# SkyTNT/midi-model

Hardware: AMD Instinct MI355X
Metric: MIDI events/sec, training step (fwd+bwd+clip+AdamW), tv2o-medium, seq=2048 (higher is better)
Workload: dtype bf16; 1 GPU; tv2o-medium bf16 training step, per-GPU batch 16 x 2048 events x 8 tokens (BASELINE.json configs[1]); random-init weights, synthetic events; global_batch=16, seq_len=2048, parallelism=dp1, accumulate_grad_batches=1, optimizer=AdamW bf16-true + global-norm clip 1.0

## Files before the change

### midi-model_amd/csrc/api.cpp

```cpp
#include <stdarg.h>
#include <stdio.h>

#include "../../include/midihip.h"

static thread_local char g_err[512] = "";

void mh_set_error(const char* fmt, ...) {
  va_list ap;
  va_start(ap, fmt);
  vsnprintf(g_err, sizeof(g_err), fmt, ap);
  va_end(ap);
}

#include <stdlib.h>
#include <string.h>
static int env_int(const char* name, int dflt) {
  const char* v = getenv(name);
  return (v && *v) ? atoi(v) : dflt;
}
thread_local int g_mh_gemm_variant = env_int("MH_GEMM", 1);
thread_local int g_mh_gemm_ablate = 0;
thread_local int g_mh_gemm_k64 = env_int("MH_GEMM_K64", 1);
thread_local int g_mh_gemm_lean_epi = env_int("MH_GEMM_LEAN_EPI", 1);
extern thread_local int g_skinny_mb, g_skinny_nbt;
extern thread_local int g_tokattn_bwd_batched;
extern thread_local int g_attn_v3, g_attn_v3_wps, g_attn_passes;

extern "C" int mh_set_option(const char* name, int value) {
  if (strcmp(name, "gemm") == 0) {
    g_mh_gemm_variant = value;
    return 0;
  }
  if (strcmp(name, "gemm_ablate") == 0) {
    g_mh_gemm_ablate = value;
    return 0;
  }
  if (strcmp(name, "gemm_k64") == 0) {
    g_mh_gemm_k64 = value;
    return 0;
  }
  if (strcmp(name, "gemm_lean_epi") == 0) {
    g_mh_gemm_lean_epi = value;
    return 0;
  }
  if (strcmp(name, "tokattn_bwd_batched") == 0) {
    g_tokattn_bwd_batched = value;
    return 0;
  }
  if (strcmp(name, "skinny_mb") == 0) {
    g_skinny_mb = value;
    return 0;
  }
  if (strcmp(name, "attn_v3") == 0) {
    g_attn_v3 = value;
    return 0;
  }
  if (strcmp(name, "attn_passes") == 0) {
    g_attn_passes = value;
    return 0;
  }
  if (strcmp(name, "attn_v3_wps") == 0) {
    g_attn_v3_wps = value;
    return 0;
  }
  if (strcmp(name, "skinny_nbt") == 0) {
    g_skinny_nbt = value;
    return 0;
  }
  mh_set_error("unknown option %s", name);
  return MH_ERR_ARG;
}
extern "C" int mh_get_option(const char* name) {
  if (strcmp(name, "gemm") == 0) return g_mh_gemm_variant;
  if (strcmp(name, "skinny_mb") == 0) return g_skinny_mb;
  if (strcmp(name, "attn_v3") == 0) return g_attn_v3;
  if (strcmp(name, "attn_v3_wps") == 0) return g_attn_v3_wps;
  if (strcmp(name, "attn_passes") == 0) return g_attn_passes;
  if (strcmp(name, "skinny_nbt") == 0) return g_skinny_nbt;
  if (strcmp(name, "gemm_k64") == 0) return g_mh_gemm_k64;
  if (strcmp(name, "gemm_ablate") == 0) return g_mh_gemm_ablate;
  if (strcmp(name, "gemm_lean_epi") == 0) return g_mh_gemm_lean_epi;
  if (strcmp(name, "tokattn_bwd_batched") == 0) return g_tokattn_bwd_batched;
  return -1;
}

extern "C" const char* mh_last_error(void) { return g_err; }
extern "C" int mh_version(void) { return 1; }
extern "C" int mh_ab_builds(void) {
#ifdef MH_AB_BUILDS
  return 1;
#else
  return 0;
#endif
}
```

### midi-model_amd/csrc/gemm_pp256.hip

```cpp
#include <limits.h>

#include <type_traits>

#include "common.h"

namespace {

__device__ __attribute__((aligned(16))) char g_zero16[16];

constexpr int QBM = 256, QBN = 256, QBK = 32;
constexpr int OP_BYTES = 256 * 64;
constexpr int STAGE_BYTES = 2 * OP_BYTES;
constexpr int NSTAGE = 4;
constexpr int LDS_BYTES = NSTAGE * STAGE_BYTES;
constexpr int NWAVE = 8;
constexpr int NI = 2;

typedef __attribute__((ext_vector_type(4))) short s16x4_t;

__device__ inline int tswz(int krow) { return (krow & 3) | ((krow >> 1) & 4); }
__device__ inline int xswz(int row) { return (0x1230 >> (((row >> 2) & 3) * 4)) & 3; }

struct StageCtx {
  const bf16* p[NI];
// ... 50 lines not shown
__device__ inline __amdgpu_buffer_rsrc_t tile_rsrc(const void* base, int64_t bytes) {
  const unsigned n = bytes <= 0 ? 0u : (bytes > 0xfffffff0ll ? 0xfffffff0u : (unsigned)bytes);
  const uint64_t b = (uint64_t)(uintptr_t)base;
  const uint64_t bu = (uint64_t)(unsigned)__builtin_amdgcn_readfirstlane((int)(unsigned)b) |
                      ((uint64_t)(unsigned)__builtin_amdgcn_readfirstlane((int)(unsigned)(b >> 32)) << 32);
  return __builtin_amdgcn_make_buffer_rsrc(reinterpret_cast<void*>((uintptr_t)bu), 0, (unsigned)__builtin_amdgcn_readfirstlane((int)n), 0x00020000);
}
template <int AUX>
__device__ inline void tile_store_(const u32x4& v, __amdgpu_buffer_rsrc_t r, unsigned voff) {
  __builtin_amdgcn_raw_buffer_store_b128(v, r, voff, 0, AUX);
}
#define tile_store(v, r, voff, aux) tile_store_<aux>(v, r, voff)
__device__ inline u32x4 as_u32x4(const bf16x8& v) {
  union {
    bf16x8 b;
    u32x4 u;
  } x;
  x.b = v;
  return x.u;
}
__device__ inline bf16x8 as_bf16x8(const u32x4& v) {
  union {
    bf16x8 b;
    u32x4 u;
  } x;
  x.u = v;
  return x.b;
}

constexpr int P8_REGION = 128 * 128;
constexpr int P8_BUF = 4 * P8_REGION;
constexpr int P8_DBG_BYTES = 8 * 2048;

template <int EPI, int ABL, bool TB>
__device__ __forceinline__ void p8_main_loop(char* smem, const bf16* __restrict__ A, int64_t lda, const bf16* __restrict__ B,
                                             int64_t ldb, int64_t M, int64_t N, int64_t m0, int64_t n0, int64_t kbeg, int64_t kend,
                                             int wave, int lane, const void* __restrict__ zero16, f32x4 (&acc)[4][8]) {
  constexpr bool TL = (ABL & 128) != 0;
  constexpr int LA = 7;
  const int grp = wave >> 2, wn = wave & 3;
  const int fi = lane & 15, fg = lane >> 4;
  const int nt = (kend > kbeg) ? (int)((kend - kbeg + 63) / 64) : 0;
  const int nreg = 4 * nt;

  int tl_n = 0;
  auto stamp = [&]() {
    if constexpr (TL) {
      const uint64_t c = __builtin_readcyclecounter();
      if (lane == 0 && tl_n < 252) *reinterpret_cast<uint64_t*>(smem + 2 * P8_BUF + wave * 2048 + tl_n * 8) = c;
      ++tl_n;
    }
  };
  auto mark = [&](int slot) {
    if constexpr (TL) {
      const uint64_t c = __builtin_readcyclecounter();
      if (lane == 0) *reinterpret_cast<uint64_t*>(smem + 2 * P8_BUF + wave * 2048 + slot * 8) = c;
    }
  };
  mark(252);

  const bf16* pa[2];
  const bf16* pb[2];
  int kla[2][2], klb[2][2];
  const int64_t hoff_a = 64 * lda, hoff_b = TB ? 32 * ldb : (EPI == 2) ? (N / 2) * ldb : 32 * ldb;
#pragma unroll
  for (int it = 0; it < 2; ++it) {
    const int lr = (wave * 2 + it) * 8 + (lane >> 3);
    const int ch = (lane & 7) ^ ((lr >> 1) & 7);
    const int64_t ra = m0 + (lr >> 6) * 128 + (lr & 63);
    pa[it] = A + (ra < M ? ra : 0) * lda + ch * 8;
    kla[0][it] = (ra < M) ? (int)kend - ch * 8 : INT_MIN;
    kla[1][it] = (ra + 64 < M) ? (int)kend - ch * 8 : INT_MIN;
    if constexpr (TB) {
      const int krow = (wave + NWAVE * it) * 2 + (lane >> 5), pc = lane & 31;
      const int lg = (pc >> 1) ^ tswz(krow);
      const int64_t r = n0 + lg * 16 + (pc & 1) * 8;
      pb[it] = B + (int64_t)krow * ldb + (r < N ? r : 0);
      klb[0][it] = (r < N) ? (int)kend - krow : INT_MIN;
      klb[1][it] = (r < N) ? (int)kend - krow - 32 : INT_MIN;
    } else {
      constexpr bool PERM = (EPI == 2 || EPI == 3);
      const int lrp = PERM ? ((lr & ~31) | (((lr & 15) >> 2) << 3) | (((lr >> 4) & 1) << 2) | (lr & 3)) : lr;
      const int64_t rb = (EPI == 2) ? n0 + lrp : n0 + (lrp >> 5) * 64 + (lrp & 31);
      const int64_t rb1 = (EPI == 2) ? rb + N / 2 : rb + 32;
      pb[it] = B + (rb < N ? rb : 0) * ldb + ch * 8;
      klb[0][it] = (rb < N) ? (int)kend - ch * 8 : INT_MIN;
      klb[1][it] = (rb1 < N) ? (int)kend - ch * 8 : INT_MIN;
    }
  }
  auto issue = [&](int s) {
    const int t = s >> 2, r = s & 3;
    const bool isb = (r == 1 || r == 2);
    const int h = (r >= 2) ? 1 : 0;
    const int slot = isb ? 2 + h : h;
    const int k0 = (int)kbeg + t * 64;
#pragma unroll
    for (int it = 0; it < 2; ++it) {
      const int piece = (TB && isb) ? wave + NWAVE * it : wave * 2 + it;
      char* dst = smem + (t & 1) * P8_BUF + slot * P8_REGION + piece * 1024;
      const bf16* p = isb ? pb[it] + (h ? hoff_b : 0) : pa[it] + (h ? hoff_a : 0);
      const int kl = isb ? klb[h][it] : kla[h][it];
      const void* src = (k0 < kl) ? (const void*)((TB && isb) ? p + (int64_t)k0 * ldb : p + k0) : zero16;
      glds16(src, dst);
    }
  };

  const int sw = (fi >> 1) & 7;
  const int la0 = (grp * 64 + fi) * 128 + ((fg ^ sw) << 4);
  const int lb0 = 2 * P8_REGION + (wn * 32 + fi) * 128 + ((fg ^ sw) << 4);
  bf16x8 fx[4][2], fw[2][2][2];
  auto read_a = [&](const char* buf, int mh) {
    if ((ABL & 2) && buf != smem) return;
#pragma unroll
    for (int m4 = 0; m4 < 4; ++m4)
#pragma unroll
      for (int kb = 0; kb < 2; ++kb)
        fx[m4][kb] = *reinterpret_cast<const bf16x8*>(buf + mh * P8_REGION + m4 * 2048 + (la0 ^ (kb << 6)));
  };
  auto read_b = [&](const char* buf, int nh) {
    if ((ABL & 2) && buf != smem) return;
#pragma unroll
    for (int n2 = 0; n2 < 2; ++n2)
#pragma unroll
      for (int kb = 0; kb < 2; ++kb) {
        if constexpr (TB) fw[nh][n2][kb] = frag<true>(buf + (2 + kb) * P8_REGION, wn * 64 + nh * 32 + n2 * 16, fi, fg);
        else fw[nh][n2][kb] = *reinterpret_cast<const bf16x8*>(buf + nh * P8_REGION + n2 * 2048 + (lb0 ^ (kb << 6)));
      }
  };
  auto mfma_q = [&](int mh, int nh) {
#pragma unroll
    for (int kb = 0; kb < 2; ++kb)
#pragma unroll
      for (int n2 = 0; n2 < 2; ++n2)
#pragma unroll
        for (int m4 = 0; m4 < 4; ++m4)
          if (!(ABL & 4))
            acc[nh * 2 + n2][mh * 4 + m4] =
                __builtin_amdgcn_mfma_f32_16x16x32_bf16(fw[nh][n2][kb], fx[m4][kb], acc[nh * 2 + n2][mh * 4 + m4], 0, 0, 0);
  };
  auto bar = [&]() {
    __builtin_amdgcn_sched_barrier(0);
    __builtin_amdgcn_s_barrier();
    __builtin_amdgcn_sched_barrier(0);
  };
  auto wait_lds = [&]() {
    asm volatile("s_waitcnt lgkmcnt(0)" ::: "memory");
    __builtin_amdgcn_sched_barrier(0);
  };
  auto wait_out = [&](int out) {
    if (out >= 4) asm volatile("s_waitcnt vmcnt(8)" ::: "memory");
    else if (out == 3) asm volatile("s_waitcnt vmcnt(6)" ::: "memory");
    else if (out == 2) asm volatile("s_waitcnt vmcnt(4)" ::: "memory");
    else if (out == 1) asm volatile("s_waitcnt vmcnt(2)" ::: "memory");
    else asm volatile("s_waitcnt vmcnt(0)" ::: "memory");
  };
  auto need = [&](int q) { return (q >> 1) * 4 + ((q & 1) ? 4 : 3); };
  auto issued_after = [&](int q) {
    const int n = (q >> 1) * 4 + ((q & 1) ? 11 : 8);
    return n < nreg ? n : nreg;
  };
  auto issue_phase = [&](int q, auto steady) {
    constexpr bool ST = decltype(steady)::value;
    if (!(ABL & 1)) {
      const int t4 = (q >> 1) * 4;
      if ((q & 1) == 0) {
        if (ST || t4 + 7 < nreg) issue(t4 + 7);
      } else {
#pragma unroll
        for (int j = 8; j < 11; ++j)
          if (ST || t4 + j < nreg) issue(t4 + j);
      }
    }
    stamp();
  };
  auto read_phase = [&](int t, int p) {
    const char* buf = smem + (t & 1) * P8_BUF;
    if (p == 0) {
      read_b(buf, 0);
      read_b(buf, 1);
      read_a(buf, 0);
    } else {
      read_a(buf, 1);
    }
    stamp();
  };
  auto load_slot = [&](int t, int p, auto steady) {
    read_phase(t, p);
    issue_phase(2 * t + p, steady);
    wait_lds();
    stamp();
  };
  auto mfma_phase = [&](int p) {
    mfma_q(p, 0);
    mfma_q(p, 1);
    stamp();
  };
  auto wait_next = [&](int q, auto steady) {
    if constexpr (decltype(steady)::value) asm volatile("s_waitcnt vmcnt(8)" ::: "memory");
    else if (q + 1 < 2 * nt) wait_out(issued_after(q) - need(q + 1));
    stamp();
  };
  auto tile_g0 = [&](int t, auto steady) {
#pragma unroll
    for (int p = 0; p < 2; ++p) {
      stamp();
      load_slot(t, p, steady);
      bar();
      stamp();
      mfma_phase(p);
      wait_next(2 * t + p, steady);
      bar();
    }
  };
  auto tile_g1 = [&](int t, auto steady) {
#pragma unroll
    for (int p = 0; p < 2; ++p) {
      stamp();
      if (2 * t + p > 0) mfma_phase(p ^ 1);
      else stamp();
      bar();
      stamp();
      load_slot(t, p, steady);
      wait_next(2 * t + p, steady);
      bar();
    }
  };

#pragma unroll
  for (int s = 0; s < LA; ++s)
    if (s < nreg) issue(s);
  if (nt > 0) wait_out((nreg < LA ? nreg : LA) - need(0));
  bar();
  mark(253);
  const int nsteady = nt > 2 ? nt - 2 : 0;
  if (grp == 0) {
    for (int t = 0; t < nsteady; ++t) tile_g0(t, std::true_type{});
    for (int t = nsteady; t < nt; ++t) tile_g0(t, std::false_type{});
  } else {
    for (int t = 0; t < nsteady; ++t) tile_g1(t, std::true_type{});
    for (int t = nsteady; t < nt; ++t) tile_g1(t, std::false_type{});
    if (nt > 0) mfma_phase(1);
  }
  mark(254);
  if constexpr (TL) {
    asm volatile("s_waitcnt lgkmcnt(0)" ::: "memory");
  }
}

constexpr int GRP_MAX = 8;
struct GrpProblem {
  const bf16* A;
  const bf16* B;
  bf16* C;
  const bf16* R;
  const bf16* wnorm;
  const bf16* W;
  float* colpart;
  int64_t lda, ldb, ldc, ldr, ldw, M, N;
  float alpha, beta;
  int tile0, tiles_n;
};
struct GrpTable {
  GrpProblem p[GRP_MAX];
  int n, nitems;
};
__host__ __device__ inline int xcd_item_of(int lin, int nitems) {
  const int q = nitems >> 3, r8 = nitems & 7, xcd = lin & 7;
  return (xcd < r8 ? xcd * (q + 1) : r8 * (q + 1) + (xcd - r8) * q) + (lin >> 3);
}
__host__ __device__ inline int grp_item_of(const GrpTable& t, int lin, int& tm, int& tn) {
  const int item = xcd_item_of(lin, t.nitems);
  int pi = 0;
#pragma unroll
  for (int j = 1; j < GRP_MAX; ++j)
    if (j < t.n && item >= t.p[j].tile0) pi = j;
  const int tiles_n = t.p[pi].tiles_n;
  const int tiles_m = (int)((t.p[pi].M + QBM - 1) / QBM);
  gemm_tile_of(item - t.p[pi].tile0, tiles_m, tiles_n, 4, tm, tn);
  return pi;
}
template <bool GRP>
struct GrpArg {
  typedef int type;
};
template <>
struct GrpArg<true> {
  typedef GrpTable type;
};

template <bool TA, bool TB, int ABL, int EPI, int ML, int NRM, bool GRP = false>
__global__ __launch_bounds__(512, 2) void gemm_pp256_kernel(const bf16* __restrict__ A, int64_t lda,
                                                            const bf16* __restrict__ B, int64_t ldb, bf16* C, int64_t ldc,
                                                            const bf16* R, int64_t ldr, int64_t M, int64_t N, int64_t K,
                                                            float alpha, float beta, int tiles_n, int nwg,
                                                            int64_t k_per_split, float* __restrict__ ws,
                                                            const void* __restrict__ zero16, float* aux, int lean_epi,
                                                            const typename GrpArg<GRP>::type gtab) {
  static_assert(NRM == 0 || (ML == 1 && ABL == 0 && !TA && (!TB || (EPI == 1 && NRM == 2))), "the norm forms ride on the K-step-64 loops only");
  static_assert(NRM != 1 || EPI == 0, "sum-of-squares partials come out of the plain epilogue");
  static_assert(!GRP || (TA && TB && ABL == 0 && EPI == 0 && ML == 0 && NRM == 0), "the grouped launch is the weight-gradient form");
  extern __shared__ __attribute__((aligned(16))) char smem[];
  const int tid = threadIdx.x, lane = tid & 63;
  const int wave = __builtin_amdgcn_readfirstlane(tid >> 6);
  const int grp = wave >> 2;
  const int wn = wave & 3;

  int zslice = 0, tm, tn;
  const bf16 *wnorm = nullptr, *Wf = nullptr;
  float* colpart = nullptr;
  int64_t ldw = 0;
  if constexpr (GRP) {
    const GrpProblem& P = gtab.p[grp_item_of(gtab, (int)blockIdx.x, tm, tn)];
    A = P.A, lda = P.lda, B = P.B, ldb = P.ldb, C = P.C, ldc = P.ldc, R = P.R, ldr = P.ldr, M = P.M, N = P.N;
    alpha = P.alpha, beta = P.beta;
    wnorm = P.wnorm, Wf = P.W, ldw = P.ldw, colpart = P.colpart;
  } else {
    const int nitems = nwg * (int)gridDim.z;
    const int lin = blockIdx.x + nwg * (int)blockIdx.z;
    const int item = xcd_item_of(lin, nitems);
    zslice = item / nwg;
    gemm_tile_of(item - zslice * nwg, nwg / tiles_n, tiles_n, 4, tm, tn);
  }
// ... 80 lines not shown
    else asm volatile("s_waitcnt vmcnt(0)" ::: "memory");
  };
  auto load_segment = [&](int t) {
    load_frags(t);
    if (t + 3 < nt && !(ABL & 1)) {
#pragma unroll
      for (int j = 0; j < 4; ++j) issue_one(t + 3, j);
    }
    asm volatile("s_waitcnt lgkmcnt(0)" ::: "memory");
    __builtin_amdgcn_sched_barrier(0);
  };
  constexpr bool MIDBAR = ((ABL & 64) != 0) == (TA || TB);
  if (grp == 0) {
    for (int t = 0; t < nt; ++t) {
      wait_step(t);
      bar();
      load_segment(t);
      if (MIDBAR) bar();
      mfma_all(t);
    }
    bar();
  } else {
    for (int t = 0; t < nt; ++t) {
      wait_step(t);
      bar();
      if (t > 0) mfma_all(t - 1);
      if (MIDBAR) bar();
      load_segment(t);
    }
    bar();
    if (nt > 0) mfma_all(nt - 1);
  }
  }

  float rs[8];
  if constexpr (NRM == 2) {
    const float* rl = reinterpret_cast<const float*>(smem + LDS_BYTES);
#pragma unroll
    for (int fm = 0; fm < 8; ++fm) rs[fm] = rl[grp * 128 + fm * 16 + fi];
  }
  const bool partial = (gridDim.z > 1);
  float* wsz = partial ? ws + (int64_t)zslice * M * N : nullptr;
  if constexpr ((ABL & 32) != 0) {
    if (acc[0][0][0] != 1.2345e38f) return;
  }
  if constexpr (EPI == 1) {
    if (lean_epi && m0 + QBM <= M && n0 + QBN <= N && ldc < (1 << 22) && ldr < (1 << 22)) {
      char* wreg = smem + wave * 16384;
      const int lrow = lane >> 3, c = lane & 7;
      const __amdgpu_buffer_rsrc_t rg = tile_rsrc(R + m0 * ldr + n0 + wn * 64, (255 * ldr + N + 64) * 2);
      const __amdgpu_buffer_rsrc_t rc = tile_rsrc(C + m0 * ldc + n0 + wn * 64, (255 * ldc + N + 64) * 2);
      const unsigned vo_r = (unsigned)(((grp * 128 + lrow) * (int)ldr + c * 8) * 2), so_r = (unsigned)ldr * 16u;
      const unsigned vo_c = (unsigned)(((grp * 128 + lrow) * (int)ldc + c * 8) * 2), so_c = (unsigned)ldc * 16u;
      const unsigned up_off = (unsigned)N * 2u;
      bf16x8 gq[2][8], uq[2][8];
      auto request = [&](int half, int i0) {
#pragma unroll
        for (int i = i0; i < i0 + 4; ++i) {
          gq[half][i] = as_bf16x8(__builtin_amdgcn_raw_buffer_load_b128(rg, vo_r, (unsigned)(half * 8 + i) * so_r, 0));
          uq[half][i] = as_bf16x8(__builtin_amdgcn_raw_buffer_load_b128(rg, vo_r, (unsigned)(half * 8 + i) * so_r + up_off, 0));
        }
      };
      request(0, 0);
      request(0, 4);
#pragma unroll
      for (int half = 0; half < 2; ++half) {
#pragma unroll
        for (int fmh = 0; fmh < 4; ++fmh)
#pragma unroll
          for (int fn = 0; fn < 4; ++fn) {
// ... 572 lines not shown
      if (partial) {
        float* dst = wsz + m * N + n;
        if (vec_ok && n + 3 < N) {
          *reinterpret_cast<f32x4*>(dst) = v;
        } else {
          for (int e = 0; e < 4 && n + e < N; ++e) dst[e] = v[e];
        }
        continue;
      }
      if (vec_ok && n + 3 < N) {
        if (R != nullptr && beta != 0.f) {
          bf16x4 rv = *reinterpret_cast<const bf16x4*>(R + m * ldr + n);
#pragma unroll
          for (int e = 0; e < 4; ++e) v[e] = alpha * v[e] + beta * (float)rv[e];
        } else {
#pragma unroll
          for (int e = 0; e < 4; ++e) v[e] = alpha * v[e];
        }
        bf16x4 o;
#pragma unroll
        for (int e = 0; e < 4; ++e) o[e] = (bf16)v[e];
        *reinterpret_cast<bf16x4*>(C + m * ldc + n) = o;
      } else {
        for (int e = 0; e < 4 && n + e < N; ++e) {
          float x = alpha * v[e];
          if (R != nullptr && beta != 0.f) x += beta * (float)R[m * ldr + n + e];
          C[m * ldc + n + e] = (bf16)x;
        }
      }
    }
  }
}

}
extern thread_local int g_mh_gemm_lean_epi;
namespace {
template <auto KERNEL>
int launch_prepare(int LDSB, void** zero16_out) {
  constexpr int MAX_DEV = 64;
  static void* zero16_of[MAX_DEV] = {};
  static bool attr_set_of[MAX_DEV] = {};
  int dev = 0;
  if (hipGetDevice(&dev) != hipSuccess || dev < 0 || dev >= MAX_DEV) {
    mh_set_error("gemm_pp256: no current device (or ordinal %d beyond %d)", dev, MAX_DEV - 1);
    return MH_ERR_LAUNCH;
  }
  void* zero16 = __atomic_load_n(&zero16_of[dev], __ATOMIC_ACQUIRE);
  if (zero16 == nullptr) {
    if (hipGetSymbolAddress(&zero16, HIP_SYMBOL(g_zero16)) != hipSuccess) {
      mh_set_error("gemm_pp256: hipGetSymbolAddress(g_zero16) failed");
      return MH_ERR_LAUNCH;
    }
    __atomic_store_n(&zero16_of[dev], zero16, __ATOMIC_RELEASE);
  }
  if (!__atomic_load_n(&attr_set_of[dev], __ATOMIC_ACQUIRE)) {
    hipError_t e = hipFuncSetAttribute(reinterpret_cast<const void*>(KERNEL), hipFuncAttributeMaxDynamicSharedMemorySize, LDSB);
    if (e != hipSuccess) {
      mh_set_error("gemm_pp256: cannot raise dynamic LDS to %d bytes: %s", LDSB, hipGetErrorString(e));
      return MH_ERR_LAUNCH;
    }
    __atomic_store_n(&attr_set_of[dev], true, __ATOMIC_RELEASE);
  }
  *zero16_out = zero16;
  return MH_OK;
}

template <bool TA, bool TB, int ABL, int EPI = 0, int ML = 0, int NRM = 0>
int launch_one(const void* A, int64_t lda, const void* B, int64_t ldb, void* C, int64_t ldc, const void* R, int64_t ldr,
               int64_t M, int64_t N, int64_t K, float alpha, float beta, int splitk, void* workspace, hipStream_t st,
               float* aux = nullptr) {
  constexpr int LDSB = LDS_BYTES + ((ABL & 128) ? P8_DBG_BYTES : 0) + (NRM == 2 ? 1024 : 0);
  void* zero16 = nullptr;
  if (int rc = launch_prepare<&gemm_pp256_kernel<TA, TB, ABL, EPI, ML, NRM>>(LDSB, &zero16)) return rc;
  const int64_t tiles_m = (M + QBM - 1) / QBM, tiles_n = (EPI == 2) ? N / 256 : (N + QBN - 1) / QBN;
  const int nwg = (int)(tiles_m * tiles_n);
  constexpr int KSTEP = (ML == 1) ? 64 : QBK;
  const int64_t kps = ((K + splitk - 1) / splitk + KSTEP - 1) / KSTEP * KSTEP;
  dim3 grid(nwg, 1, splitk);
  gemm_pp256_kernel<TA, TB, ABL, EPI, ML, NRM><<<grid, 512, LDSB, st>>>((const bf16*)A, lda, (const bf16*)B, ldb, (bf16*)C, ldc,
                                                          (const bf16*)R, ldr, M, N, K, alpha, beta, (int)tiles_n, nwg, kps,
                                                          (float*)workspace, zero16, aux, g_mh_gemm_lean_epi, 0);
  MH_LAUNCH_CHECK();
  return MH_OK;
}

void grp_table_of(const mh_wgrad_problem* p, int n, GrpTable& t) {
  t.n = n;
  int tile0 = 0;
  for (int j = 0; j < GRP_MAX; ++j) {
    GrpProblem& g = t.p[j];
    if (j >= n) {
      g = GrpProblem{};
      g.tile0 = INT_MAX;
      continue;
    }
    g.A = (const bf16*)p[j].dz, g.lda = p[j].lddz, g.B = (const bf16*)p[j].x, g.ldb = p[j].ldx;
    g.C = (bf16*)p[j].dw, g.ldc = p[j].lddw, g.R = (const bf16*)p[j].R, g.ldr = p[j].ldr;
    g.wnorm = (const bf16*)p[j].wnorm, g.W = (const bf16*)p[j].W, g.ldw = p[j].ldw, g.colpart = p[j].colpart;
    g.M = p[j].N, g.N = p[j].K_out, g.alpha = p[j].alpha, g.beta = p[j].beta;
    g.tile0 = tile0;
    g.tiles_n = (int)((g.N + QBN - 1) / QBN);
    tile0 += (int)((g.M + QBM - 1) / QBM) * g.tiles_n;
  }
  t.nitems = tile0;
}
// ... 156 lines not shown
```

Before: 366,800 events/s.

## Add persistent 256x256 GEMM kernel that prefetches the next tile during epilogue

Adds a persistent variant of the pp256 GEMM that launches one workgroup per CU and loops over tiles. While a tile's epilogue runs through a small per-wave LDS staging region, the global-to-LDS loads for the next tile are already issued, and the vmcnt waits are adjusted to count the epilogue stores still in flight. The aim is to hide the epilogue and per-tile launch/prologue latency behind the next tile's loads. It is enabled by default for selected EPI/TB/K classes, with an environment switch to turn it off. The cost is extra LDS use, more complicated waitcnt accounting, and possible load imbalance when the tile count is not a multiple of the CU count.

```diff
diff --git a/midi-model_amd/csrc/api.cpp b/midi-model_amd/csrc/api.cpp
--- a/midi-model_amd/csrc/api.cpp
+++ b/midi-model_amd/csrc/api.cpp
@@ -22,6 +22,8 @@
 thread_local int g_mh_gemm_ablate = 0;
 thread_local int g_mh_gemm_k64 = env_int("MH_GEMM_K64", 1);
 thread_local int g_mh_gemm_lean_epi = env_int("MH_GEMM_LEAN_EPI", 1);
+thread_local int g_mh_gemm_persist = env_int("MH_GEMM_PERSIST", 1);
+thread_local int g_mh_gemm_persist_wgs = env_int("MH_GEMM_PERSIST_WGS", 0);
 extern thread_local int g_skinny_mb, g_skinny_nbt;
 extern thread_local int g_tokattn_bwd_batched;
 extern thread_local int g_attn_v3, g_attn_v3_wps, g_attn_passes;
@@ -41,6 +43,14 @@
   }
   if (strcmp(name, "gemm_lean_epi") == 0) {
     g_mh_gemm_lean_epi = value;
+    return 0;
+  }
+  if (strcmp(name, "gemm_persist") == 0) {
+    g_mh_gemm_persist = value;
+    return 0;
+  }
+  if (strcmp(name, "gemm_persist_wgs") == 0) {
+    g_mh_gemm_persist_wgs = value;
     return 0;
   }
   if (strcmp(name, "tokattn_bwd_batched") == 0) {
@@ -80,6 +90,8 @@
   if (strcmp(name, "gemm_k64") == 0) return g_mh_gemm_k64;
   if (strcmp(name, "gemm_ablate") == 0) return g_mh_gemm_ablate;
   if (strcmp(name, "gemm_lean_epi") == 0) return g_mh_gemm_lean_epi;
+  if (strcmp(name, "gemm_persist") == 0) return g_mh_gemm_persist;
+  if (strcmp(name, "gemm_persist_wgs") == 0) return g_mh_gemm_persist_wgs;
   if (strcmp(name, "tokattn_bwd_batched") == 0) return g_tokattn_bwd_batched;
   return -1;
 }
diff --git a/midi-model_amd/csrc/gemm_pp256.hip b/midi-model_amd/csrc/gemm_pp256.hip
--- a/midi-model_amd/csrc/gemm_pp256.hip
+++ b/midi-model_amd/csrc/gemm_pp256.hip
@@ -106,68 +106,55 @@
 constexpr int P8_BUF = 4 * P8_REGION;
 constexpr int P8_DBG_BYTES = 8 * 2048;
 
-template <int EPI, int ABL, bool TB>
-__device__ __forceinline__ void p8_main_loop(char* smem, const bf16* __restrict__ A, int64_t lda, const bf16* __restrict__ B,
-                                             int64_t ldb, int64_t M, int64_t N, int64_t m0, int64_t n0, int64_t kbeg, int64_t kend,
-                                             int wave, int lane, const void* __restrict__ zero16, f32x4 (&acc)[4][8]) {
-  constexpr bool TL = (ABL & 128) != 0;
-  constexpr int LA = 7;
-  const int grp = wave >> 2, wn = wave & 3;
-  const int fi = lane & 15, fg = lane >> 4;
-  const int nt = (kend > kbeg) ? (int)((kend - kbeg + 63) / 64) : 0;
-  const int nreg = 4 * nt;
-
-  int tl_n = 0;
-  auto stamp = [&]() {
-    if constexpr (TL) {
-      const uint64_t c = __builtin_readcyclecounter();
-      if (lane == 0 && tl_n < 252) *reinterpret_cast<uint64_t*>(smem + 2 * P8_BUF + wave * 2048 + tl_n * 8) = c;
-      ++tl_n;
-    }
-  };
-  auto mark = [&](int slot) {
-    if constexpr (TL) {
-      const uint64_t c = __builtin_readcyclecounter();
-      if (lane == 0) *reinterpret_cast<uint64_t*>(smem + 2 * P8_BUF + wave * 2048 + slot * 8) = c;
-    }
-  };
-  mark(252);
-
+constexpr int P8_LA = 7;
+
+template <int EPI, bool TB>
+struct P8Feed {
+  char* smem;
+  const void* zero16;
   const bf16* pa[2];
   const bf16* pb[2];
   int kla[2][2], klb[2][2];
-  const int64_t hoff_a = 64 * lda, hoff_b = TB ? 32 * ldb : (EPI == 2) ? (N / 2) * ldb : 32 * ldb;
-#pragma unroll
-  for (int it = 0; it < 2; ++it) {
-    const int lr = (wave * 2 + it) * 8 + (lane >> 3);
-    const int ch = (lane & 7) ^ ((lr >> 1) & 7);
-    const int64_t ra = m0 + (lr >> 6) * 128 + (lr & 63);
-    pa[it] = A + (ra < M ? ra : 0) * lda + ch * 8;
-    kla[0][it] = (ra < M) ? (int)kend - ch * 8 : INT_MIN;
-    kla[1][it] = (ra + 64 < M) ? (int)kend - ch * 8 : INT_MIN;
-    if constexpr (TB) {
-      const int krow = (wave + NWAVE * it) * 2 + (lane >> 5), pc = lane & 31;
-      const int lg = (pc >> 1) ^ tswz(krow);
-      const int64_t r = n0 + lg * 16 + (pc & 1) * 8;
-      pb[it] = B + (int64_t)krow * ldb + (r < N ? r : 0);
-      klb[0][it] = (r < N) ? (int)kend - krow : INT_MIN;
-      klb[1][it] = (r < N) ? (int)kend - krow - 32 : INT_MIN;
-    } else {
-      constexpr bool PERM = (EPI == 2 || EPI == 3);
-      const int lrp = PERM ? ((lr & ~31) | (((lr & 15) >> 2) << 3) | (((lr >> 4) & 1) << 2) | (lr & 3)) : lr;
-      const int64_t rb = (EPI == 2) ? n0 + lrp : n0 + (lrp >> 5) * 64 + (lrp & 31);
-      const int64_t rb1 = (EPI == 2) ? rb + N / 2 : rb + 32;
-      pb[it] = B + (rb < N ? rb : 0) * ldb + ch * 8;
-      klb[0][it] = (rb < N) ? (int)kend - ch * 8 : INT_MIN;
-      klb[1][it] = (rb1 < N) ? (int)kend - ch * 8 : INT_MIN;
-    }
-  }
-  auto issue = [&](int s) {
+  int64_t hoff_a, hoff_b, ldb;
+  int kbeg, wave;
+
+  __device__ __forceinline__ void init(char* smem_, const bf16* __restrict__ A, int64_t lda, const bf16* __restrict__ B, int64_t ldb_,
+                                       int64_t M, int64_t N, int64_t m0, int64_t n0, int64_t kbeg_, int64_t kend, int wave_, int lane,
+                                       const void* __restrict__ zero16_) {
+    smem = smem_, zero16 = zero16_, ldb = ldb_, kbeg = (int)kbeg_, wave = wave_;
+    hoff_a = 64 * lda, hoff_b = TB ? 32 * ldb : (EPI == 2) ? (N / 2) * ldb : 32 * ldb;
+#pragma unroll
+    for (int it = 0; it < 2; ++it) {
+      const int lr = (wave * 2 + it) * 8 + (lane >> 3);
+      const int ch = (lane & 7) ^ ((lr >> 1) & 7);
+      const int64_t ra = m0 + (lr >> 6) * 128 + (lr & 63);
+      pa[it] = A + (ra < M ? ra : 0) * lda + ch * 8;
+      kla[0][it] = (ra < M) ? (int)kend - ch * 8 : INT_MIN;
+      kla[1][it] = (ra + 64 < M) ? (int)kend - ch * 8 : INT_MIN;
+      if constexpr (TB) {
+        const int krow = (wave + NWAVE * it) * 2 + (lane >> 5), pc = lane & 31;
+        const int lg = (pc >> 1) ^ tswz(krow);
+        const int64_t r = n0 + lg * 16 + (pc & 1) * 8;
+        pb[it] = B + (int64_t)krow * ldb + (r < N ? r : 0);
+        klb[0][it] = (r < N) ? (int)kend - krow : INT_MIN;
+        klb[1][it] = (r < N) ? (int)kend - krow - 32 : INT_MIN;
+      } else {
+        constexpr bool PERM = (EPI == 2 || EPI == 3);
+        const int lrp = PERM ? ((lr & ~31) | (((lr & 15) >> 2) << 3) | (((lr >> 4) & 1) << 2) | (lr & 3)) : lr;
+        const int64_t rb = (EPI == 2) ? n0 + lrp : n0 + (lrp >> 5) * 64 + (lrp & 31);
+        const int64_t rb1 = (EPI == 2) ? rb + N / 2 : rb + 32;
+        pb[it] = B + (rb < N ? rb : 0) * ldb + ch * 8;
+        klb[0][it] = (rb < N) ? (int)kend - ch * 8 : INT_MIN;
+        klb[1][it] = (rb1 < N) ? (int)kend - ch * 8 : INT_MIN;
+      }
+    }
+  }
+  __device__ __forceinline__ void issue(int s) const {
     const int t = s >> 2, r = s & 3;
     const bool isb = (r == 1 || r == 2);
     const int h = (r >= 2) ? 1 : 0;
     const int slot = isb ? 2 + h : h;
-    const int k0 = (int)kbeg + t * 64;
+    const int k0 = kbeg + t * 64;
 #pragma unroll
     for (int it = 0; it < 2; ++it) {
       const int piece = (TB && isb) ? wave + NWAVE * it : wave * 2 + it;
@@ -177,7 +164,53 @@
       const void* src = (k0 < kl) ? (const void*)((TB && isb) ? p + (int64_t)k0 * ldb : p + k0) : zero16;
       glds16(src, dst);
     }
-  };
+  }
+};
+
+template <int EPI, bool TB>
+__device__ __forceinline__ void p8_prefetch(char* smem, const bf16* __restrict__ A, int64_t lda, const bf16* __restrict__ B, int64_t ldb,
+                                            int64_t M, int64_t N, int64_t m0, int64_t n0, int64_t K, int wave, int lane,
+                                            const void* __restrict__ zero16) {
+  P8Feed<EPI, TB> feed;
+  feed.init(smem, A, lda, B, ldb, M, N, m0, n0, 0, K, wave, lane, zero16);
+  const int nreg = 4 * (int)((K + 63) / 64);
+#pragma unroll
+  for (int s = 0; s < P8_LA; ++s)
+    if (s < nreg) feed.issue(s);
+}
+
+template <int EPI, int ABL, bool TB, int EV = -1>
+__device__ __forceinline__ void p8_main_loop(char* smem, const bf16* __restrict__ A, int64_t lda, const bf16* __restrict__ B,
+                                             int64_t ldb, int64_t M, int64_t N, int64_t m0, int64_t n0, int64_t kbeg, int64_t kend,
+                                             int wave, int lane, const void* __restrict__ zero16, f32x4 (&acc)[4][8],
+                                             bool behind = false) {
+  constexpr bool TL = (ABL & 128) != 0;
+  constexpr int LA = P8_LA;
+  static_assert(EV < 0 || (ABL == 0 && 8 + EV < 64), "vmcnt is a 6-bit count");
+  const int grp = wave >> 2, wn = wave & 3;
+  const int fi = lane & 15, fg = lane >> 4;
+  const int nt = (kend > kbeg) ? (int)((kend - kbeg + 63) / 64) : 0;
+  const int nreg = 4 * nt;
+
+  int tl_n = 0;
+  auto stamp = [&]() {
+    if constexpr (TL) {
+      const uint64_t c = __builtin_readcyclecounter();
+      if (lane == 0 && tl_n < 252) *reinterpret_cast<uint64_t*>(smem + 2 * P8_BUF + wave * 2048 + tl_n * 8) = c;
+      ++tl_n;
+    }
+  };
+  auto mark = [&](int slot) {
+    if constexpr (TL) {
+      const uint64_t c = __builtin_readcyclecounter();
+      if (lane == 0) *reinterpret_cast<uint64_t*>(smem + 2 * P8_BUF + wave * 2048 + slot * 8) = c;
+    }
+  };
+  mark(252);
+
+  P8Feed<EPI, TB> feed;
+  feed.init(smem, A, lda, B, ldb, M, N, m0, n0, kbeg, kend, wave, lane, zero16);
+  auto issue = [&](int s) { feed.issue(s); };
 
   const int sw = (fi >> 1) & 7;
   const int la0 = (grp * 64 + fi) * 128 + ((fg ^ sw) << 4);
@@ -221,7 +254,17 @@
     asm volatile("s_waitcnt lgkmcnt(0)" ::: "memory");
     __builtin_amdgcn_sched_barrier(0);
   };
-  auto wait_out = [&](int out) {
+  auto wait_out = [&](int out, bool extra = false) {
+    if constexpr (EV > 0) {
+      if (extra) {
+        if (out >= 4) asm volatile("s_waitcnt vmcnt(%0)" ::"n"(8 + EV) : "memory");
+        else if (out == 3) asm volatile("s_waitcnt vmcnt(%0)" ::"n"(6 + EV) : "memory");
+        else if (out == 2) asm volatile("s_waitcnt vmcnt(%0)" ::"n"(4 + EV) : "memory");
+        else if (out == 1) asm volatile("s_waitcnt vmcnt(%0)" ::"n"(2 + EV) : "memory");
+        else asm volatile("s_waitcnt vmcnt(%0)" ::"n"(EV) : "memory");
+        return;
+      }
+    }
     if (out >= 4) asm volatile("s_waitcnt vmcnt(8)" ::: "memory");
     else if (out == 3) asm volatile("s_waitcnt vmcnt(6)" ::: "memory");
     else if (out == 2) asm volatile("s_waitcnt vmcnt(4)" ::: "memory");
@@ -270,8 +313,9 @@
     stamp();
   };
   auto wait_next = [&](int q, auto steady) {
-    if constexpr (decltype(steady)::value) asm volatile("s_waitcnt vmcnt(8)" ::: "memory");
-    else if (q + 1 < 2 * nt) wait_out(issued_after(q) - need(q + 1));
+    const bool extra = EV > 0 && behind && q < 2;
+    if constexpr (decltype(steady)::value) wait_out(4, extra);
+    else if (q + 1 < 2 * nt) wait_out(issued_after(q) - need(q + 1), extra);
     stamp();
   };
   auto tile_g0 = [&](int t, auto steady) {
@@ -300,10 +344,12 @@
     }
   };
 
-#pragma unroll
-  for (int s = 0; s < LA; ++s)
-    if (s < nreg) issue(s);
-  if (nt > 0) wait_out((nreg < LA ? nreg : LA) - need(0));
+  if constexpr (EV < 0) {
+#pragma unroll
+    for (int s = 0; s < LA; ++s)
+      if (s < nreg) issue(s);
+  }
+  if (nt > 0) wait_out((nreg < LA ? nreg : LA) - need(0), EV > 0 && behind);
   bar();
   mark(253);
   const int nsteady = nt > 2 ? nt - 2 : 0;
@@ -362,6 +408,12 @@
   typedef GrpTable type;
 };
 
+template <int EPI, int ABL, int ML, int NRM, bool GRP>
+__device__ __forceinline__ void pp256_epilogue(char* smem, const float* rl, f32x4 (&acc)[4][8], bf16* C, int64_t ldc, const bf16* R,
+                                               int64_t ldr, int64_t M, int64_t N, float alpha, float beta, int64_t m0, int64_t n0, int tm,
+                                               int zslice, float* __restrict__ ws, float* aux, int lean_epi, int wave, int lane,
+                                               const bf16* wnorm, const bf16* Wf, int64_t ldw, float* colpart);
+
 template <bool TA, bool TB, int ABL, int EPI, int ML, int NRM, bool GRP = false>
 __global__ __launch_bounds__(512, 2) void gemm_pp256_kernel(const bf16* __restrict__ A, int64_t lda,
                                                             const bf16* __restrict__ B, int64_t ldb, bf16* C, int64_t ldc,
@@ -508,10 +560,19 @@
     if (nt > 0) mfma_all(nt - 1);
   }
   }
-
+  pp256_epilogue<EPI, ABL, ML, NRM, GRP>(smem, reinterpret_cast<const float*>(smem + LDS_BYTES), acc, C, ldc, R, ldr, M, N, alpha, beta, m0, n0,
+                                         tm, zslice, ws, aux, lean_epi, wave, lane, wnorm, Wf, ldw, colpart);
+}
+
+template <int EPI, int ABL, int ML, int NRM, bool GRP>
+__device__ __forceinline__ void pp256_epilogue(char* smem, const float* rl, f32x4 (&acc)[4][8], bf16* C, int64_t ldc, const bf16* R,
+                                               int64_t ldr, int64_t M, int64_t N, float alpha, float beta, int64_t m0, int64_t n0, int tm,
+                                               int zslice, float* __restrict__ ws, float* aux, int lean_epi, int wave, int lane,
+                                               const bf16* wnorm, const bf16* Wf, int64_t ldw, float* colpart) {
+  const int grp = wave >> 2, wn = wave & 3;
+  const int fi = lane & 15, fg = lane >> 4;
   float rs[8];
   if constexpr (NRM == 2) {
-    const float* rl = reinterpret_cast<const float*>(smem + LDS_BYTES);
 #pragma unroll
     for (int fm = 0; fm < 8; ++fm) rs[fm] = rl[grp * 128 + fm * 16 + fi];
   }
@@ -1150,8 +1211,333 @@
   }
 }
 
+constexpr int P8_TURN_LO = P8_BUF + P8_REGION;
+constexpr int P8_TURN_HI = LDS_BYTES;
+constexpr int P8_RSTD = LDS_BYTES + P8_REGION;
+constexpr int P8_PERSIST_LDS = P8_RSTD + 2048;
+template <int EPI, int NRM>
+constexpr int p8_epi_stores() {
+  return EPI == 1 ? 32 : EPI == 2 ? 24 : (EPI == 0 && NRM == 1) ? 32 : 16;
+}
+
+template <int EPI, int NRM>
+__device__ __forceinline__ void p8_epilogue_turn4k(char* wreg, const float* rl, f32x4 (&acc)[4][8], bf16* C, int64_t ldc, const bf16* R,
+                                                   int64_t ldr, int64_t M, int64_t N, float alpha, float beta, int64_t m0, int64_t n0,
+                                                   float* aux, int wave, int lane) {
+  const int grp = wave >> 2, wn = wave & 3;
+  const int fi = lane & 15, fg = lane >> 4;
+  float rs[8];
+  if constexpr (NRM == 2) {
+#pragma unroll
+    for (int fm = 0; fm < 8; ++fm) rs[fm] = rl[grp * 128 + fm * 16 + fi];
+  }
+  auto put_f32 = [&](int fm) {
+#pragma unroll
+    for (int fn = 0; fn < 4; ++fn) {
+      const int ch = fn * 4 + fg;
+      f32x4 t4 = acc[fn][fm];
+      if constexpr (NRM == 2) t4 *= rs[fm];
+      *reinterpret_cast<f32x4*>(wreg + fi * 256 + ((ch ^ fi) << 4)) = t4;
+    }
+  };
+  if constexpr (EPI == 1) {
+    const int lrow = lane >> 3, c = lane & 7;
+    const __amdgpu_buffer_rsrc_t rg = tile_rsrc(R + m0 * ldr + n0 + wn * 64, (255 * ldr + N + 64) * 2);
+    const __amdgpu_buffer_rsrc_t rc = tile_rsrc(C + m0 * ldc + n0 + wn * 64, (255 * ldc + N + 64) * 2);
+    const unsigned vo_r = (unsigned)(((grp * 128 + lrow) * (int)ldr + c * 8) * 2), so_r = (unsigned)ldr * 16u;
+    const unsigned vo_c = (unsigned)(((grp * 128 + lrow) * (int)ldc + c * 8) * 2), so_c = (unsigned)ldc * 16u;
+    const unsigned up_off = (unsigned)N * 2u;
+    bf16x8 gq[16], uq[16];
+    auto request = [&](int i0) {
+#pragma unroll
+      for (int i = i0; i < i0 + 4; ++i) {
+        gq[i] = as_bf16x8(__builtin_amdgcn_raw_buffer_load_b128(rg, vo_r, (unsigned)i * so_r, 0));
+        uq[i] = as_bf16x8(__builtin_amdgcn_raw_buffer_load_b128(rg, vo_r, (unsigned)i * so_r + up_off, 0));
+      }
+    };
+    request(0);
+    request(4);
+#pragma unroll
+    for (int fm = 0; fm < 8; ++fm) {
+      put_f32(fm);
+#pragma unroll
+      for (int i2 = 0; i2 < 2; ++i2) {
+        const int i = fm * 2 + i2, row = i2 * 8 + lrow;
+        if (i == 2) request(8);
+        if (i == 6) request(12);
+        const f32x4 lo = *reinterpret_cast<const f32x4*>(wreg + row * 256 + (((2 * c) ^ row) << 4));
+        const f32x4 hi = *reinterpret_cast<const f32x4*>(wreg + row * 256 + (((2 * c + 1) ^ row) << 4));
+        const float v[8] = {lo[0], lo[1], lo[2], lo[3], hi[0], hi[1], hi[2], hi[3]};
+        float dv[8], g[8], u[8], dg[8], du[8];
+        expand8_bf16(cvt8_bf16(v), dv);
+        expand8_bf16(gq[i], g);
+        expand8_bf16(uq[i], u);
+        mh_dswiglu8(dv, g, u, dg, du);
+        const unsigned so = (unsigned)i * so_c;
+        tile_store(as_u32x4(cvt8_bf16(dg)), rc, vo_c + so, 2 );
+        tile_store(as_u32x4(cvt8_bf16(du)), rc, vo_c + so + up_off, 2);
+      }
+    }
+  } else if constexpr (EPI == 2) {
+    const int64_t I = N >> 1, colw = n0 + wn * 32;
+    bf16* act = const_cast<bf16*>(R);
+    const __amdgpu_buffer_rsrc_t ra = tile_rsrc(act + m0 * ldr + colw, (255 * ldr + 32) * 2);
+    const __amdgpu_buffer_rsrc_t rc = tile_rsrc(C + m0 * ldc + colw, (255 * ldc + I + 32) * 2);
+    const int r4 = lane >> 2, c4 = lane & 3;
+    const unsigned vo_a = (unsigned)(((grp * 128 + r4) * (int)ldr + c4 * 8) * 2), so_a = (unsigned)ldr * 32u;
+    const unsigned vo_c = (unsigned)(((grp * 128 + r4) * (int)ldc + c4 * 8) * 2), so_c = (unsigned)ldc * 32u;
+#pragma unroll
+    for (int fm = 0; fm < 8; ++fm) {
+      float gf[8], uf[8];
+#pragma unroll
+      for (int e = 0; e < 4; ++e) {
+        gf[e] = acc[0][fm][e];
+        gf[4 + e] = acc[1][fm][e];
+        uf[e] = acc[2][fm][e];
+        uf[4 + e] = acc[3][fm][e];
+      }
+      if constexpr (NRM == 2) {
+#pragma unroll
+        for (int e = 0; e < 8; ++e) {
+          gf[e] *= rs[fm];
+          uf[e] *= rs[fm];
+        }
+      }
+      const bf16x8 og = cvt8_bf16(gf), ou = cvt8_bf16(uf);
+      float gr[8], ur[8], sv[8], sr[8], av[8];
+      expand8_bf16(og, gr);
+      expand8_bf16(ou, ur);
+      mh_silu8(gr, sv);
+      expand8_bf16(cvt8_bf16(sv), sr);
+#pragma unroll
+      for (int e = 0; e < 8; ++e) av[e] = sr[e] * ur[e];
+      const bf16x8 oa = cvt8_bf16(av);
+      const int off = fi * 64 + ((fg ^ ((fi >> 1) & 3)) << 4), off2 = r4 * 64 + ((c4 ^ ((r4 >> 1) & 3)) << 4);
+      *reinterpret_cast<u32x4*>(wreg + off) = as_u32x4(oa);
+      *reinterpret_cast<u32x4*>(wreg + 1024 + off) = as_u32x4(og);
+      *reinterpret_cast<u32x4*>(wreg + 2048 + off) = as_u32x4(ou);
+      const u32x4 va = *reinterpret_cast<const u32x4*>(wreg + off2);
+      tile_store(va, ra, vo_a + (unsigned)fm * so_a, 0);
+      const u32x4 vg = *reinterpret_cast<const u32x4*>(wreg + 1024 + off2);
+      const u32x4 vu = *reinterpret_cast<const u32x4*>(wreg + 2048 + off2);
+      tile_store(vg, rc, vo_c + (unsigned)fm * so_c, 0);
+      tile_store(vu, rc, vo_c + (unsigned)fm * so_c + (unsigned)I * 2u, 0);
+    }
+  } else if constexpr (EPI == 3) {
+    const int64_t nw = n0 + wn * 64;
+    const bool rot = nw < 2 * (N / 3);
+    const bf16* tab = R;
+    const unsigned S_ = (unsigned)(ldr & 0xffffffff), pos0 = (unsigned)(ldr >> 32);
+    const unsigned mrow = (unsigned)m0 + (unsigned)(grp * 128 + fi);
+    const unsigned p0 = mrow % S_;
+    bf16x8 cq[8], s1q[8], s2q[8];
+    if (rot) {
+#pragma unroll
+      for (int fm = 0; fm < 8; ++fm) {
+        unsigned pf = p0 + 16u * fm;
+        if (S_ >= 128u) pf = (pf >= S_) ? pf - S_ : pf;
+        else pf %= S_;
+        const bf16* t = tab + (size_t)(pos0 + pf) * 96 + fg * 8;
+        cq[fm] = *reinterpret_cast<const bf16x8*>(t);
+        s1q[fm] = *reinterpret_cast<const bf16x8*>(t + 32);
+        s2q[fm] = *reinterpret_cast<const bf16x8*>(t + 64);
+      }
+    }
+    const __amdgpu_buffer_rsrc_t rc = tile_rsrc(C + m0 * ldc + nw, (255 * ldc + 64) * 2);
+    const int r8 = lane >> 3, c8 = lane & 7;
+    const unsigned vo = (unsigned)(((grp * 128 + r8) * (int)ldc + c8 * 8) * 2), so8 = (unsigned)ldc * 16u;
+#pragma unroll
+    for (int p = 0; p < 4; ++p) {
+#pragma unroll
+      for (int f2 = 0; f2 < 2; ++f2) {
+        const int fm = p * 2 + f2;
+        float x1[8], x2[8];
+#pragma unroll
+        for (int e = 0; e < 4; ++e) {
+          x1[e] = acc[0][fm][e];
+          x1[4 + e] = acc[1][fm][e];
+          x2[e] = acc[2][fm][e];
+          x2[4 + e] = acc[3][fm][e];
+        }
+        if constexpr (NRM == 2) {
+#pragma unroll
+          for (int e = 0; e < 8; ++e) {
+            x1[e] *= rs[fm];
+            x2[e] *= rs[fm];
+          }
+        }
+        bf16x8 b1 = cvt8_bf16(x1), b2 = cvt8_bf16(x2);
+        if (rot) {
+          float v1[8], v2[8], cf[8], s1[8], s2[8], o1[8], o2[8];
+          expand8_bf16(b1, v1);
+          expand8_bf16(b2, v2);
+          expand8_bf16(cq[fm], cf);
+          expand8_bf16(s1q[fm], s1);
+          expand8_bf16(s2q[fm], s2);
+#pragma unroll
+          for (int e = 0; e < 8; ++e) {
+            o1[e] = __builtin_fmaf(v1[e], cf[e], v2[e] * s1[e]);
+            o2[e] = __builtin_fmaf(v2[e], cf[e], v1[e] * s2[e]);
+          }
+          b1 = cvt8_bf16(o1);
+          b2 = cvt8_bf16(o2);
+        }
+        const int row = f2 * 16 + fi;
+        *reinterpret_cast<u32x4*>(wreg + row * 128 + ((fg ^ (row & 7)) << 4)) = as_u32x4(b1);
+        *reinterpret_cast<u32x4*>(wreg + row * 128 + (((4 + fg) ^ (row & 7)) << 4)) = as_u32x4(b2);
+      }
+#pragma unroll
+      for (int i4 = 0; i4 < 4; ++i4) {
+        const int row = i4 * 8 + r8;
+        const u32x4 v = *reinterpret_cast<const u32x4*>(wreg + row * 128 + ((c8 ^ (row & 7)) << 4));
+        tile_store(v, rc, vo + (unsigned)(p * 4 + i4) * so8, 2 );
+      }
+    }
+  } else {
+    const int lrow = lane >> 3, c = lane & 7;
+    const bool use_r = (R != nullptr && beta != 0.f);
+    const __amdgpu_buffer_rsrc_t rc = tile_rsrc(C + m0 * ldc + n0 + wn * 64, (255 * ldc + 64) * 2);
+    const __amdgpu_buffer_rsrc_t rr = tile_rsrc(use_r ? R + m0 * ldr + n0 + wn * 64 : nullptr, use_r ? (255 * ldr + 64) * 2 : 0);
+    const unsigned vo_c = (unsigned)(((grp * 128 + lrow) * (int)ldc + c * 8) * 2), so_c = (unsigned)ldc * 16u;
+    const unsigned vo_r = (unsigned)(((grp * 128 + lrow) * (int)ldr + c * 8) * 2), so_r = (unsigned)ldr * 16u;
+    float* auxp = nullptr;
+    if constexpr (NRM == 1) auxp = aux + ((n0 + wn * 64) >> 6) * M + m0 + grp * 128 + lrow;
+    auto turn = [&](auto with_r) {
+      constexpr bool use_r = decltype(with_r)::value;
+      bf16x8 rv[16];
+      if (use_r) {
+#pragma unroll
+        for (int i = 0; i < 16; ++i) rv[i] = as_bf16x8(__builtin_amdgcn_raw_buffer_load_b128(rr, vo_r, (unsigned)i * so_r, 0));
+      }
+#pragma unroll
+      for (int fm = 0; fm < 8; ++fm) {
+        put_f32(fm);
+#pragma unroll
+        for (int i2 = 0; i2 < 2; ++i2) {
+          const int i = fm * 2 + i2, row = i2 * 8 + lrow;
+          const f32x4 lo = *reinterpret_cast<const f32x4*>(wreg + row * 256 + (((2 * c) ^ row) << 4));
+          const f32x4 hi = *reinterpret_cast<const f32x4*>(wreg + row * 256 + (((2 * c + 1) ^ row) << 4));
+          float v[8] = {lo[0], lo[1], lo[2], lo[3], hi[0], hi[1], hi[2], hi[3]};
+          if (use_r) {
+#pragma unroll
+            for (int e = 0; e < 8; ++e) v[e] = alpha * v[e] + beta * (float)rv[i][e];
+          } else {
+#pragma unroll
+            for (int e = 0; e < 8; ++e) v[e] = alpha * v[e];
+          }
+          bf16x8 o;
+#pragma unroll
+          for (int e = 0; e < 8; ++e) o[e] = (bf16)v[e];
+          tile_store(as_u32x4(o), rc, vo_c + (unsigned)i * so_c, 2 );
+          if constexpr (NRM == 1) {
+            union {
+              bf16x8 v8;
+              bf16x2 h[4];
+            } u;
+            u.v8 = o;
+            float ss = 0.f;
+#pragma unroll
+            for (int e = 0; e < 4; ++e) ss = __builtin_amdgcn_fdot2_f32_bf16(u.h[e], u.h[e], ss, false);
+            ss += dpp_move<0xB1>(ss);
+            ss += dpp_move<0x4E>(ss);
+            ss += dpp_move<0x141>(ss);
+            if (c == 0) auxp[i * 8] = ss;
+          }
+        }
+      }
+    };
+    if (__builtin_amdgcn_readfirstlane((int)use_r)) turn(std::true_type{});
+    else turn(std::false_type{});
+  }
+}
+
+template <bool TB, int EPI, int NRM>
+__global__ __launch_bounds__(512, 2) void gemm_pp256_persist_kernel(const bf16* __restrict__ A, int64_t lda, const bf16* __restrict__ B,
+                                                                    int64_t ldb, bf16* C, int64_t ldc, const bf16* R, int64_t ldr,
+                                                                    int64_t M, int64_t N, int64_t K, float alpha, float beta,
+                                                                    int tiles_n, int nwg, const void* __restrict__ zero16, float* aux,
+                                                                    int lean_epi) {
+  static_assert(NRM == 0 || (!TB || (EPI == 1 && NRM == 2)), "as gemm_pp256_kernel");
+  extern __shared__ __attribute__((aligned(16))) char smem[];
+  constexpr int EV = p8_epi_stores<EPI, NRM>();
+  const int tid = threadIdx.x, lane = tid & 63;
+  const int wave = __builtin_amdgcn_readfirstlane(tid >> 6);
+  char* wturn = smem + (wave < 4 ? P8_TURN_LO + wave * 4096 : P8_TURN_HI + (wave - 4) * 4096);
+  int64_t m0, n0;
+  auto tile_of = [&](int lin) {
+    int tm, tn;
+    gemm_tile_of(xcd_item_of(lin, nwg), nwg / tiles_n, tiles_n, 4, tm, tn);
+    m0 = (int64_t)tm * QBM, n0 = (int64_t)tn * (EPI == 2 ? 128 : QBN);
+  };
+  auto rstd_of = [&](int j) { return smem + P8_RSTD + (j & 1) * 1024; };
+  auto fresh = [](int v) {
+    asm volatile("" : "+v"(v));
+    return v;
+  };
+  auto prefetch = [&](int j) {
+    const int lane = fresh(tid & 63);
+    if constexpr (NRM == 2) {
+      if (wave == 0) {
+        const int64_t r = m0 + lane * 4;
+        glds16((r + 4 <= M) ? (const void*)(aux + r) : zero16, rstd_of(j));
+      }
+    }
+    p8_prefetch<EPI, TB>(smem, A, lda, B, ldb, M, N, m0, n0, K, wave, lane, zero16);
+  };
+  auto interior = [&]() {
+    bool in = m0 + QBM <= M && n0 + QBN <= N && ldc < (1 << 22);
+    if constexpr (EPI == 0) {
+      const bool use_r = (R != nullptr && beta != 0.f);
+      in = in && lean_epi && ldr < (1 << 22) && (ldc & 7) == 0 && ((uintptr_t)C & 15) == 0 &&
+           (!use_r || ((ldr & 7) == 0 && ((uintptr_t)R & 15) == 0));
+    }
+    if constexpr (EPI == 1) in = in && lean_epi && ldr < (1 << 22);
+    if constexpr (EPI == 2) in = m0 + QBM <= M && C != nullptr;
+    return in;
+  };
+  int lin = blockIdx.x;
+  tile_of(lin);
+  prefetch(0);
+  bool behind = false;
+  for (int j = 0;; ++j) {
+    f32x4 acc[4][8];
+#pragma unroll
+    for (int a = 0; a < 4; ++a)
+#pragma unroll
+      for (int b = 0; b < 8; ++b) acc[a][b] = f32x4{0.f, 0.f, 0.f, 0.f};
+    p8_main_loop<EPI, 0, TB, EV>(smem, A, lda, B, ldb, M, N, m0, n0, 0, K, wave, fresh(lane), zero16, acc, behind);
+    const int next = lin + (int)gridDim.x;
+    const bool more = next < nwg;
+    const int64_t cm0 = m0, cn0 = n0;
+    if (interior()) {
+      if (more) {
+        tile_of(next);
+        prefetch(j + 1);
+      }
+      p8_epilogue_turn4k<EPI, NRM>(wturn, reinterpret_cast<const float*>(rstd_of(j)), acc, C, ldc, R, ldr, M, N, alpha, beta, cm0, cn0,
+                                   aux, wave, fresh(lane));
+      if (!more) break;
+      behind = true;
+    } else {
+      pp256_epilogue<EPI, 0, 1, NRM, false>(smem, reinterpret_cast<const float*>(rstd_of(j)), acc, C, ldc, R, ldr, M, N, alpha, beta, cm0,
+                                            cn0, 0, 0, nullptr, aux, lean_epi, wave, fresh(lane), nullptr, nullptr, 0, nullptr);
+      if (!more) break;
+      asm volatile("s_waitcnt vmcnt(0) lgkmcnt(0)" ::: "memory");
+      __builtin_amdgcn_sched_barrier(0);
+      __builtin_amdgcn_s_barrier();
+      __builtin_amdgcn_sched_barrier(0);
+      tile_of(next);
+      prefetch(j + 1);
+      behind = false;
+    }
+    lin = next;
+  }
+}
+
 }
 extern thread_local int g_mh_gemm_lean_epi;
+extern thread_local int g_mh_gemm_persist;
+extern thread_local int g_mh_gemm_persist_wgs;
 namespace {
 template <auto KERNEL>
 int launch_prepare(int LDSB, void** zero16_out) {
@@ -1183,12 +1569,50 @@
   return MH_OK;
 }
 
+int persist_grid(int64_t tiles) {
+  constexpr int MAX_DEV = 64;
+  static int cus_of[MAX_DEV] = {};
+  int dev = 0;
+  if (hipGetDevice(&dev) != hipSuccess || dev < 0 || dev >= MAX_DEV) return 0;
+  int cus = __atomic_load_n(&cus_of[dev], __ATOMIC_ACQUIRE);
+  if (cus == 0) {
+    if (hipDeviceGetAttribute(&cus, hipDeviceAttributeMultiprocessorCount, dev) != hipSuccess || cus <= 0) return 0;
+    __atomic_store_n(&cus_of[dev], cus, __ATOMIC_RELEASE);
+  }
+  int grid = cus;
+  if (g_mh_gemm_persist_wgs > 0 && g_mh_gemm_persist_wgs < grid) grid = g_mh_gemm_persist_wgs;
+  return tiles < grid ? (int)tiles : grid;
+}
+
+template <bool TB, int EPI, int NRM>
+bool persist_class(int64_t K) {
+  if (g_mh_gemm_persist != 1) return g_mh_gemm_persist > 1;
+  if (EPI == 1 || EPI == 2) return true;
+  if (EPI == 0 && TB) return K >= 2048;
+  if (EPI == 0 && NRM == 1) return K <= 2048;
+  if (EPI == 0 && NRM == 0) return true;
+  return false;
+}
+
 template <bool TA, bool TB, int ABL, int EPI = 0, int ML = 0, int NRM = 0>
 int launch_one(const void* A, int64_t lda, const void* B, int64_t ldb, void* C, int64_t ldc, const void* R, int64_t ldr,
                int64_t M, int64_t N, int64_t K, float alpha, float beta, int splitk, void* workspace, hipStream_t st,
                float* aux = nullptr) {
   constexpr int LDSB = LDS_BYTES + ((ABL & 128) ? P8_DBG_BYTES : 0) + (NRM == 2 ? 1024 : 0);
   void* zero16 = nullptr;
+  if constexpr (ML == 1 && ABL == 0) {
+    const int64_t tiles = ((M + QBM - 1) / QBM) * ((EPI == 2) ? N / 256 : (N + QBN - 1) / QBN);
+    const int grid = persist_grid(tiles);
+    if (persist_class<TB, EPI, NRM>(K) && splitk == 1 && grid > 0 && tiles > grid && tiles < INT_MAX && !(EPI == 2 && C == nullptr)) {
+      if (int rc = launch_prepare<&gemm_pp256_persist_kernel<TB, EPI, NRM>>(P8_PERSIST_LDS, &zero16)) return rc;
+      const int tn = (int)((EPI == 2) ? N / 256 : (N + QBN - 1) / QBN);
+      gemm_pp256_persist_kernel<TB, EPI, NRM><<<dim3(grid, 1, 1), 512, P8_PERSIST_LDS, st>>>(
+          (const bf16*)A, lda, (const bf16*)B, ldb, (bf16*)C, ldc, (const bf16*)R, ldr, M, N, K, alpha, beta, tn, (int)tiles, zero16, aux,
+          g_mh_gemm_lean_epi);
+      MH_LAUNCH_CHECK();
+      return MH_OK;
+    }
+  }
   if (int rc = launch_prepare<&gemm_pp256_kernel<TA, TB, ABL, EPI, ML, NRM>>(LDSB, &zero16)) return rc;
   const int64_t tiles_m = (M + QBM - 1) / QBM, tiles_n = (EPI == 2) ? N / 256 : (N + QBN - 1) / QBN;
   const int nwg = (int)(tiles_m * tiles_n);
```

Result: no change. 368,800 events/s, median of 6 (+0.5%).
